# shanjiayao/PTT

Measured on AMD Instinct MI355X. Metric: tracklet frames/sec (hot path: PointNet++ SA stack + Point-Track-Transformer blocks), higher is better.
Workload: dtype f32

## Files before the change

include/ptt_hip.h:

```cpp
#ifndef PTT_HIP_H
#define PTT_HIP_H

#include <stddef.h>
#include <stdint.h>

#ifdef __cplusplus
extern "C" {
#endif

#define PTT_ABI_VERSION 21

enum {
    PTT_OK = 0,
    PTT_EINVAL = -1,
    PTT_EUNSUPPORTED = -2,
    PTT_ELAUNCH = -3,
    PTT_EWORKSPACE = -4
};

typedef void* ptt_stream_t;

int ptt_version(void);
const char* ptt_error_name(int code);
const char* ptt_last_error_string(void);

int ptt_fps_f32(const float* xyz, int B, int N, int npoint, int32_t* idx_out,
                ptt_stream_t stream);
int ptt_fps_ws_f32(const float* xyz, int B, int N, int npoint, int32_t* idx_out, float* workspace,
                   size_t workspace_elems, ptt_stream_t stream);

int ptt_gather_f32(const float* feat, const int32_t* idx, int B, int C, int N, int M,
                   float* out, ptt_stream_t stream);
int ptt_gather_grad_f32(const float* grad_out, const int32_t* idx, int B, int C, int N,
// ... 81 lines not shown
    float radius;
    int32_t ns, M, normalize_xyz, pro_relu;
} ptt_row_job;
int ptt_row_jobs_f32(const ptt_row_job* jobs, int n_jobs, ptt_stream_t stream);

typedef struct ptt_sa_desc {
    const float* xyz;
    const float* new_xyz;
    const int32_t* idx;
    const float* feat;
    int64_t feat_sb, feat_sc, feat_sn;
    float* out;
    int64_t out_sb, out_sc, out_sm;
    int B, N, M, nsample, C;
    float radius;
    int use_xyz;
    int normalize_xyz;
    int n_layers;
    ptt_sa_layer layers[PTT_SA_MAX_LAYERS];
    const float* l0_point_term;
    const float* l0_xyz_weight;
    int l0_channels;
    int l0_relu;
} ptt_sa_desc;

int ptt_sa_fused_fwd_f32(const ptt_sa_desc* d, ptt_stream_t stream);

typedef struct ptt_xcorr_desc {
    const float* cos_t;
    const float* P;
    const float* w_sim;
    const float* scale0;
    const float* shift0;
    float* out;
    int64_t out_sb, out_sc, out_sn;
    float* sim_out;
    int B, Ns, Nt, C0;
    int n_layers;
    ptt_sa_layer layers[PTT_SA_MAX_LAYERS];
    int32_t split; int64_t out_sh;
    const float* search_feat; const float* templ_feat;
    int64_t s_sb, s_sn, t_sb, t_sn;
    int C; float eps;
} ptt_xcorr_desc;

int ptt_xcorr_fused_fwd_f32(const ptt_xcorr_desc* d, ptt_stream_t stream);

int ptt_cosine_map_f32(const float* search_feat, int64_t s_sb, int64_t s_sn, int64_t s_sc, const float* templ_feat,
                       int64_t t_sb, int64_t t_sn, int64_t t_sc, int B, int Ns, int Nt, int C, float eps,
// ... 299 lines not shown
```

ptt_amd/_lib.py:

```python
import ctypes
import os
from ctypes import POINTER, Structure, c_char_p, c_double, c_float, c_int, c_int32, c_int64, c_longlong, c_size_t, c_uint32, c_void_p

_HERE = os.path.dirname(os.path.abspath(__file__))
LIB_PATH = os.path.join(_HERE, "lib", "libptt_hip.so")

PTT_SA_MAX_LAYERS = 4
ABI_VERSION = 21

EXPORTS = [
    "ptt_version", "ptt_error_name", "ptt_last_error_string",
    "ptt_fps_f32", "ptt_fps_ws_f32", "ptt_spatial_order_f32", "ptt_ball_query_grid_workspace", "ptt_ball_query_grid_f32",
    "ptt_centres_ball_query_grid_f32", "ptt_gather_f32", "ptt_gather_grad_f32", "ptt_select_centres_f32", "ptt_ball_query_f32",
    "ptt_group_f32", "ptt_group_grad_f32", "ptt_scatter_add_det_workspace", "ptt_scatter_add_det_f32",
    "ptt_knn_f32", "ptt_knn_rel_f32",
    "ptt_packed_weight_elems", "ptt_pack_weight_f32", "ptt_pack_weight_rot_f32", "ptt_linear_f32",
    "ptt_sa_fused_fwd_f32", "ptt_xcorr_fused_fwd_f32", "ptt_cosine_map_f32", "ptt_pt_attn_pair_f32",
    "ptt_crop_compact_f32", "ptt_regularize_f32", "ptt_mt19937_fill", "ptt_select_box_f32",
    "ptt_track_crop_bounds", "ptt_track_box_by_offset",
    "ptt_bn_stats_workspace", "ptt_bn_stats_f32", "ptt_bn_apply_f32", "ptt_bn_bwd_f32", "ptt_pool_rows_f32",
    "ptt_pool_rows_bwd_f32", "ptt_linear_wgrad_workspace", "ptt_linear_wgrad_f32",
    "ptt_pack_weight_strided_f32", "ptt_linear_batched_f32", "ptt_softmax_rows_f32",
    "ptt_gather_rows_f32", "ptt_scatter_csr_i32", "ptt_scatter_rows_csr_f32",
    "ptt_pt_pair_input_f32", "ptt_pt_attn_train_fwd_f32", "ptt_pt_attn_train_bwd_f32", "ptt_linear_act_in_f32",
    "ptt_centres_ball_query_f32",
    "ptt_bn_sums_f64", "ptt_bn_finish_f64", "ptt_bn_bwd_sums_f64", "ptt_bn_bwd_apply_f32",
    "ptt_rows_mlp_f32",
    "ptt_rows_gemm_supported", "ptt_rows_gemm_stat_chunks", "ptt_rows_gemm_f32", "ptt_rows_gemm_masked_f32", "ptt_bn_finish_partials_f32",
    "ptt_bn_sums_partials_f64", "ptt_linear_wgrad2_workspace", "ptt_linear_wgrad2_f32",
    "ptt_bn_bwd_pooled_f32", "ptt_bn_bwd_pooled_sums_f64", "ptt_bn_bwd_pooled_apply_f32",
    "ptt_pt_pair_input_ld_f32", "ptt_pt_attn_fwd_ld_f32",
    "ptt_rows_gemm_bnbwd_f32", "ptt_bn_bwd_from_partials_f32", "ptt_bn_bwd_sums_partials_f64",
    "ptt_bn_bwd_consts_f32", "ptt_bn_bwd_pooled_consts_f32", "ptt_rows_gemm_bnbwd_fused_supported", "ptt_rows_gemm_bnbwd_fused_f32",
    "ptt_bn_update_running_f32", "ptt_xcorr_z0_f32", "ptt_xcorr_z0_stat_chunks", "ptt_xcorr_z0_stats_f32", "ptt_xcorr_z0_bnbwd_f32", "ptt_xcorr_z0_bwd_workspace", "ptt_xcorr_z0_bwd_f32",
    "ptt_bn_stats_train_f32", "ptt_bn_finish_partials_train_f32", "ptt_pack_weights_f32",
    "ptt_sa_z0_rows_f32",
    "ptt_row_jobs_f32", "ptt_point_jobs_f32", "ptt_fps_ball_knn_f32", "ptt_crop_compact_host_f32", "ptt_crop_regularize_f32", "ptt_colsum_workspace", "ptt_colsum_f32", "ptt_rows_gemm_pool_supported", "ptt_rows_gemm_pool_f32", "ptt_pool_select_f32", "ptt_sa_z0_rows_stat_chunks", "ptt_sa_z0_rows_stats_f32",
    "ptt_track_losses_f32", "ptt_track_losses_bwd_f32", "ptt_adam_chunk_elems", "ptt_adam_clip_step_f32", "ptt_adam_clip_step_dev_f32",
    "ptt_linear_wgrad_partials_f32", "ptt_linear_wgrad2_partials_f32", "ptt_colsum_partials_f32", "ptt_grad_finish_f32",
    "ptt_rows_gemm_rsum16_supported", "ptt_rows_gemm_rsum16_f32", "ptt_scatter_rows_csr_sub_f32",
    "ptt_unit_rows_f32", "ptt_cos_bwd_rows_f32", "ptt_track_select_update", "ptt_sa_z0_bnbwd_workspace", "ptt_sa_z0_bnbwd_f32",
]
PTT_MAX_SEGMENTS = 4


class CropJob(Structure):
    _fields_ = [("points", c_void_p), ("ld", c_int64),
                ("lo1", c_double * 3), ("hi1", c_double * 3), ("trans", c_double * 3), ("rot", c_double * 9),
                ("lo2", c_double * 3), ("hi2", c_double * 3),
                ("out", c_void_p), ("count", c_void_p), ("n_points", c_int32), ("capacity", c_int32),
                ("label_out", c_void_p), ("ltrans", c_double * 3), ("lrot", c_double * 9), ("llo", c_double * 3), ("lhi", c_double * 3)]


class RegularizeJob(Structure):
    _fields_ = [("seg", c_void_p * PTT_MAX_SEGMENTS), ("seg_count", c_void_p * PTT_MAX_SEGMENTS),
                ("seg_capacity", c_int32 * PTT_MAX_SEGMENTS), ("out", c_void_p), ("info", c_void_p),
                ("n_seg", c_int32), ("input_size", c_int32)]



class BnTrainTail(Structure):
    _fields_ = [("gamma", c_void_p), ("beta", c_void_p), ("act_a", c_void_p), ("act_b", c_void_p),
                ("running_mean", c_void_p), ("running_var", c_void_p), ("num_batches_tracked", c_void_p), ("momentum", c_float)]

# ... 45 lines not shown

class GradSegment(Structure):
    _fields_ = [("dst", c_int64), ("n", c_int32), ("cols", c_int32), ("ld", c_int32), ("job0", c_int32), ("njobs", c_int32), ("out", c_int32),
                ("vec", c_int32), ("reserved", c_int32)]


class AdamHyper(Structure):
    _fields_ = [("beta1", c_float), ("beta2", c_float), ("one_minus_beta1", c_float), ("one_minus_beta2", c_float), ("eps", c_float), ("step_size", c_float), ("bias2_sqrt", c_float),
                ("weight_decay", c_float), ("max_norm", c_float), ("write_clipped", c_int32)]


class SaLayer(Structure):
    _fields_ = [("Wpacked", c_void_p), ("scale", c_void_p), ("shift", c_void_p),
                ("Cin", c_int), ("Cout", c_int), ("relu", c_int)]


class SaDesc(Structure):
    _fields_ = [("xyz", c_void_p), ("new_xyz", c_void_p), ("idx", c_void_p), ("feat", c_void_p),
                ("feat_sb", c_int64), ("feat_sc", c_int64), ("feat_sn", c_int64),
                ("out", c_void_p), ("out_sb", c_int64), ("out_sc", c_int64), ("out_sm", c_int64),
                ("B", c_int), ("N", c_int), ("M", c_int), ("nsample", c_int), ("C", c_int),
                ("radius", c_float), ("use_xyz", c_int), ("normalize_xyz", c_int), ("n_layers", c_int),
                ("layers", SaLayer * PTT_SA_MAX_LAYERS),
                ("l0_point_term", c_void_p), ("l0_xyz_weight", c_void_p), ("l0_channels", c_int), ("l0_relu", c_int)]


class XcorrDesc(Structure):
    _fields_ = [("cos_t", c_void_p), ("P", c_void_p), ("w_sim", c_void_p), ("scale0", c_void_p), ("shift0", c_void_p),
                ("out", c_void_p), ("out_sb", c_int64), ("out_sc", c_int64), ("out_sn", c_int64),
                ("sim_out", c_void_p),
                ("B", c_int), ("Ns", c_int), ("Nt", c_int), ("C0", c_int),
                ("n_layers", c_int), ("layers", SaLayer * PTT_SA_MAX_LAYERS),
                ("split", c_int32), ("out_sh", c_int64), ("search_feat", c_void_p), ("templ_feat", c_void_p),
                ("s_sb", c_int64), ("s_sn", c_int64), ("t_sb", c_int64), ("t_sn", c_int64), ("C", c_int), ("eps", c_float)]


class AttnDesc(Structure):
    _fields_ = [("xyz", c_void_p), ("rel", c_void_p), ("knn", c_void_p), ("qkv", c_void_p),
                ("Wd1p", c_void_p), ("Wd2p", c_void_p), ("bd2", c_void_p),
                ("Wg1p", c_void_p), ("bg1", c_void_p), ("Wg2p", c_void_p), ("bg2", c_void_p),
                ("res", c_void_p), ("attn", c_void_p),
                ("B", c_int), ("N", c_int), ("k", c_int), ("D", c_int), ("order", c_void_p)]


_lib = None


# ... 107 lines not shown
        "ptt_bn_bwd_pooled_apply_f32": [vp, i, vp, i, vp, i, vp, vp, vp, vp, vp, vp, i, i, vp, i, vp, vp, vp],
        "ptt_row_jobs_f32": [POINTER(RowJob), i, vp],
        "ptt_point_jobs_f32": [POINTER(PointJob), i, vp],
        "ptt_fps_ball_knn_f32": [vp, i, i, i, f, i, i, vp, vp, vp, vp, vp, vp, vp],
    }
    for name, args in sigs.items():
        fn = getattr(lib, name)
        fn.restype = c_int
        fn.argtypes = args
    lib.ptt_packed_weight_elems.restype = c_size_t
    lib.ptt_packed_weight_elems.argtypes = [i, i]
    lib.ptt_scatter_add_det_workspace.restype = c_size_t
    lib.ptt_scatter_add_det_workspace.argtypes = [i, i, i]
    lib.ptt_ball_query_grid_workspace.restype = c_size_t
    lib.ptt_ball_query_grid_workspace.argtypes = [i, i]
    lib.ptt_bn_stats_workspace.restype = c_size_t
    lib.ptt_bn_stats_workspace.argtypes = [i, i]
    lib.ptt_linear_wgrad_workspace.restype = c_size_t
    lib.ptt_linear_wgrad_workspace.argtypes = [i, i, i]
    lib.ptt_xcorr_z0_bwd_workspace.restype = c_size_t
    lib.ptt_xcorr_z0_bwd_workspace.argtypes = [i, i, i]
    lib.ptt_sa_z0_bnbwd_workspace.restype = c_size_t
    lib.ptt_sa_z0_bnbwd_workspace.argtypes = [c_longlong, i]
    lib.ptt_adam_chunk_elems.restype = c_int
    lib.ptt_adam_chunk_elems.argtypes = []
    lib.ptt_colsum_workspace.restype = c_size_t
    lib.ptt_colsum_workspace.argtypes = [i, i]
    lib.ptt_linear_wgrad2_workspace.restype = c_size_t
    lib.ptt_linear_wgrad2_workspace.argtypes = [i, i, i]


def lib():
    global _lib
    if _lib is None:
        if not os.path.exists(LIB_PATH):
            raise RuntimeError(
                "ptt_amd: %s is missing — build it with `python -m ptt_amd.build` "
                "(hipcc --offload-arch=gfx950); there is no CPU fallback" % LIB_PATH)
        import torch
        try:
            loaded = ctypes.CDLL(LIB_PATH)
        except OSError as e:
            raise RuntimeError("ptt_amd: cannot load %s: %s" % (LIB_PATH, e))
        _declare(loaded)
        if loaded.ptt_version() != ABI_VERSION:
            raise RuntimeError("ptt_amd: %s has ABI version %d, this package expects %d — rebuild it with "
# ... 11 lines not shown
```

ptt_amd/csrc/mfma_ops.hip:

```cpp
#include <math.h>
#include <stdlib.h>
#include <string.h>
#include "common.h"
#include "mfma_common.h"

#ifndef PTT_PAIR_PF
#define PTT_PAIR_PF 1
#endif
#ifndef PTT_GATHER_BATCH
#define PTT_GATHER_BATCH 16
#endif
#ifndef PTT_SA_WAVES
#define PTT_SA_WAVES 2
#endif

namespace ptt {

#ifdef PTT_DEV
#define PTT_STAMP(i) do { if (p.dbg && threadIdx.x == 0 && blockIdx.x < 4096) p.dbg[blockIdx.x * 8 + (i)] = __builtin_readcyclecounter(); } while (0)
#else
#define PTT_STAMP(i) do { } while (0)
#endif

__device__ __forceinline__ void stagger_second_slot(int first_wave_blocks, int quanta) {
// ... 399 lines not shown
    const float sc = p.scale ? p.scale[col] : 1.f;
    const float sh = p.shift ? p.shift[col] : 0.f;
#pragma unroll
    for (int r = 0; r < 16; ++r) {
        const int gr = row0 + tile_row(r, half);
        if (gr >= p.rows) continue;
        float y = (acc[r] + Rs[(cw * 16 + r) * 64 + lane]) * sc + sh;
        if (p.relu) y = fmaxf(y, 0.f);
        if (p.residual) y += p.residual[(size_t)gr * p.ldr + col];
        p.out[(size_t)gr * p.ldo + col] = y;
    }
}

struct SaLayerDev { const float* Wp; const float* scale; const float* shift; int Cin, Cout, relu, nkb, NT; };
struct SaParams {
    const float* xyz; const float* new_xyz; const int32_t* idx; const float* feat; float* out;
    long long fsb, fsc, fsn, osb, osc, osm;
    int B, N, M, C, use_xyz, normalize, n_layers, ldk, K0, first_wave, stagger, vec_gather;
    int tiles, chunk;
    int hoist, l0_relu;
    const float* wx;
    float radius;
    long long* dbg;
    SaLayerDev L[PTT_SA_MAX_LAYERS];
};

struct RowsMlpParams {
    const float* X; const float* residual; float* out;
    int rows, K0, ldx, ldr, ldo, n_layers, ldk, vec_in;
    SaLayerDev L[PTT_SA_MAX_LAYERS];
};

__global__ __launch_bounds__(256, 2) void rows_mlp_kernel(RowsMlpParams p) {
    extern __shared__ __attribute__((aligned(16))) float smem[];
    float* Xs = smem;
    const int t = threadIdx.x, lane = t & 63, w = t >> 6, half = lane >> 5;
    const int row0 = blockIdx.x * 32;
    f32x4 pw[3];
    float psh[3];
    auto prefetch = [&](const SaLayerDev& L) {
        const f32x4* bp = reinterpret_cast<const f32x4*>(L.Wp) + (size_t)w * 64 + lane;
#pragma unroll
        for (int u = 0; u < 3; ++u) {
            psh[u] = 0.f;
            if (w + 4 * u < L.NT) {
                pw[u] = bp[(size_t)u * 4 * 64];
// ... 783 lines not shown
            } else {
                float m0 = y[0], m1 = y[8];
#pragma unroll
                for (int r = 1; r < 8; ++r) { m0 = fmaxf(m0, y[r]); m1 = fmaxf(m1, y[8 + r]); }
                m0 = max_halves(m0);
                m1 = max_halves(m1);
                if (L.relu) { m0 = fmaxf(m0, 0.f); m1 = fmaxf(m1, 0.f); }
                if (half == 0) {
                    if (2 * rt < ncentres) {
                        const int c = centre0 + 2 * rt; const int b = c / p.M, mm = c - b * p.M;
                        p.out[b * p.osb + col * p.osc + mm * p.osm] = m0;
                    }
                    if (2 * rt + 1 < ncentres) {
                        const int c = centre0 + 2 * rt + 1; const int b = c / p.M, mm = c - b * p.M;
                        p.out[b * p.osb + col * p.osc + mm * p.osm] = m1;
                    }
                }
            }
        }
    }
    __builtin_amdgcn_wave_barrier();
}

#ifndef PTT_SAL_WGS
#define PTT_SAL_WGS 1
#endif
#ifndef PTT_SAL_WAVES
#define PTT_SAL_WAVES 12
#endif
__global__ __launch_bounds__(64 * PTT_SAL_WAVES) __attribute__((amdgpu_waves_per_eu(PTT_SAL_WAVES * PTT_SAL_WGS / 4)))
void sa_lds_kernel(SaParams p) {
    extern __shared__ __attribute__((aligned(16))) float smem[];
    float* W1 = smem;
    float* W2 = smem + 4096;
    const int t = threadIdx.x, lane = t & 63, half = lane >> 5, col = lane & 31;
    const int w = __builtin_amdgcn_readfirstlane(t >> 6);
    {
        const f32x4* g1 = reinterpret_cast<const f32x4*>(p.L[1].Wp);
        const f32x4* g2 = reinterpret_cast<const f32x4*>(p.L[2].Wp);
        f32x4* s1 = reinterpret_cast<f32x4*>(W1);
        f32x4* s2 = reinterpret_cast<f32x4*>(W2);
        const int nthr = (int)blockDim.x;
        for (int i = t; i < 1024; i += nthr) s1[i] = g1[i];
        for (int i = t; i < 2048; i += nthr) s2[i] = g2[i];
    }
    float* cst = smem + 4096 + 8192 + w * 640 + lane;
#pragma unroll
    for (int u = 0; u < 2; ++u) {
        const f32x4 f = reinterpret_cast<const f32x4*>(p.L[0].Wp)[u * 64 + col];
        const float s0 = p.L[0].shift ? p.L[0].shift[u * 32 + col] : 0.f;
        cst[(0 + u) * 64] = half ? f[1] : f[0];
        cst[(2 + u) * 64] = half ? s0 : f[2];
        cst[(4 + u) * 64] = p.L[1].shift ? p.L[1].shift[u * 32 + col] : 0.f;
    }
#pragma unroll
    for (int u = 0; u < 4; ++u) cst[(6 + u) * 64] = p.L[2].shift ? p.L[2].shift[u * 32 + col] : 0.f;
    const float one_zero = half ? 0.f : 1.f, one_hi = 1.f;
    __syncthreads();
    const int total = p.B * p.M, M = p.M, N = p.N;
    const int gw = logical_block() * ((int)blockDim.x >> 6) + w;
    const int c0 = gw * p.chunk, c1 = min(total, c0 + p.chunk);
    if (c0 >= c1) return;
    const float rdiv = p.normalize ? p.radius : 1.0f;
    const int osb = (int)p.osb, osm = (int)p.osm, osc = (int)p.osc;
    const f32x16 zero16 = {0.f, 0.f, 0.f, 0.f, 0.f, 0.f, 0.f, 0.f, 0.f, 0.f, 0.f, 0.f, 0.f, 0.f, 0.f, 0.f};
    const float* a1p = W1 + lane * 4;
    const float* b2p = W2 + lane * 4;
    const __amdgpu_buffer_rsrc_t rx = weight_rsrc(p.xyz);

    SasCentre ce;
    ce.c = c0; ce.b = c0 / M; ce.m = c0 - ce.b * M;
    int n_cur = p.idx[(size_t)c0 * 32 + col];
    float px, py, pz, cx, cy, cz;
    {
        const size_t flat = (size_t)ce.b * N + n_cur;
        px = p.xyz[flat * 3]; py = p.xyz[flat * 3 + 1]; pz = p.xyz[flat * 3 + 2];
        cx = p.new_xyz[(size_t)c0 * 3]; cy = p.new_xyz[(size_t)c0 * 3 + 1]; cz = p.new_xyz[(size_t)c0 * 3 + 2];
    }
    for (int c = c0; c < c1; ++c) {
        SasCentre nx = ce;
        if (c + 1 < c1) nx.advance(1, M);
        const int n_next = p.idx[(size_t)nx.c * 32 + col];
        f32x4 wa[2], wn[2];
#pragma unroll
        for (int u = 0; u < 2; ++u) wa[u] = *reinterpret_cast<const f32x4*>(a1p + u * 256);
        const float dx = (px - cx) / rdiv, dy = (py - cy) / rdiv, dz = (pz - cz) / rdiv;
        __builtin_amdgcn_sched_barrier(0);
        f32x16 h0[2];
        {
            const float k0 = half ? dy : dx, k1 = half ? one_hi : dz;
#pragma unroll
            for (int u = 0; u < 2; ++u) h0[u] = __builtin_amdgcn_mfma_f32_32x32x2f32(cst[(0 + u) * 64], k0, zero16, 0, 0, 0);
#pragma unroll
            for (int u = 0; u < 2; ++u) h0[u] = __builtin_amdgcn_mfma_f32_32x32x2f32(cst[(2 + u) * 64], k1, h0[u], 0, 0, 0);
#pragma unroll
            for (int u = 0; u < 2; ++u)
#pragma unroll
                for (int r = 0; r < 16; ++r) h0[u][r] = fmaxf(h0[u][r], 0.f);
        }
        f32x16 h1[2];
        f32x4 wb[4], wm[4];
        {
#pragma unroll
            for (int u = 0; u < 2; ++u) h1[u] = __builtin_amdgcn_mfma_f32_32x32x2f32(cst[(4 + u) * 64], one_zero, zero16, 0, 0, 0);
#pragma unroll
// ... 1 lines not shown
                if (kb < 7) {
#pragma unroll
                    for (int u = 0; u < 2; ++u) wn[u] = *reinterpret_cast<const f32x4*>(a1p + ((kb + 1) * 2 + u) * 256);
                } else {
#pragma unroll
                    for (int u = 0; u < 4; ++u) wb[u] = *reinterpret_cast<const f32x4*>(b2p + u * 256);
                }
                __builtin_amdgcn_sched_barrier(0);
#pragma unroll
                for (int j = 0; j < 4; ++j)
#pragma unroll
                    for (int u = 0; u < 2; ++u)
                        h1[u] = __builtin_amdgcn_mfma_f32_32x32x2f32(wa[u][j], h0[kb >> 2][(kb & 3) * 4 + j], h1[u], 0, 0, 0);
                __builtin_amdgcn_sched_barrier(0);
#pragma unroll
                for (int u = 0; u < 2; ++u) wa[u] = wn[u];
            }
#pragma unroll
            for (int u = 0; u < 2; ++u)
#pragma unroll
                for (int r = 0; r < 16; ++r) h1[u][r] = fmaxf(h1[u][r], 0.f);
        }
        {
            const int off = (nx.b * N + n_next) * 12;
            px = __builtin_bit_cast(float, __builtin_amdgcn_raw_buffer_load_b32(rx, off, 0, 0));
            py = __builtin_bit_cast(float, __builtin_amdgcn_raw_buffer_load_b32(rx, off + 4, 0, 0));
            pz = __builtin_bit_cast(float, __builtin_amdgcn_raw_buffer_load_b32(rx, off + 8, 0, 0));
            cx = p.new_xyz[(size_t)nx.c * 3]; cy = p.new_xyz[(size_t)nx.c * 3 + 1]; cz = p.new_xyz[(size_t)nx.c * 3 + 2];
        }
        __builtin_amdgcn_sched_barrier(0);
        {
            f32x16 acc[4];
#pragma unroll
            for (int kb = 0; kb < 8; ++kb) {
                if (kb < 7) {
#pragma unroll
                    for (int u = 0; u < 4; ++u) wm[u] = *reinterpret_cast<const f32x4*>(b2p + ((kb + 1) * 4 + u) * 256);
                }
                __builtin_amdgcn_sched_barrier(0);
#pragma unroll
                for (int j = 0; j < 4; ++j)
#pragma unroll
                    for (int u = 0; u < 4; ++u)
                        acc[u] = __builtin_amdgcn_mfma_f32_32x32x2f32(h1[kb >> 2][(kb & 3) * 4 + j], wb[u][j],
                                                                       (kb == 0 && j == 0) ? zero16 : acc[u], 0, 0, 0);
                __builtin_amdgcn_sched_barrier(0);
#pragma unroll
                for (int u = 0; u < 4; ++u) wb[u] = wm[u];
            }
            float* o = p.out + (ce.b * osb + ce.m * osm);
#pragma unroll
            for (int u = 0; u < 4; ++u) {
                const float mx = sas_pool(acc[u], cst[(6 + u) * 64], p.L[2].relu);
                if (half == 0) o[(u * 32 + col) * osc] = mx;
            }
        }
        ce = nx;
    }
}

template <int NS, int RT>
__global__ __launch_bounds__(256, 2) void sa_wave_kernel(SaParams p) {
    extern __shared__ __attribute__((aligned(16))) float smem[];
    constexpr int CPW = 32 * RT / NS;
    const int t = threadIdx.x, lane = t & 63, w = t >> 6;
    float* Xw = smem + w * 32 * RT * p.ldk;
    const int total_centres = p.B * p.M;
    const int centre0 = (logical_block() * 4 + w) * CPW;
    if (centre0 >= total_centres) return;
    const int ncentres = min(CPW, total_centres - centre0);

#pragma unroll
    for (int rt = 0; rt < RT; ++rt) sa_gather_rows<NS, 32>(p, Xw, rt * 32, centre0, lane);
    __builtin_amdgcn_wave_barrier();

    for (int l = 0; l < p.n_layers; ++l) {
        const SaLayerDev& L = p.L[l];
        const bool last = (l == p.n_layers - 1);
#define PTT_WAVE_LAYER(CTV)                                                                         \
        { if (L.scale) sa_wave_layer<NS, CTV, true, RT>(p, L, last, Xw, lane, centre0, ncentres);       \
// ... 335 lines not shown
        const ptt_sa_layer& s = layers[l];
        const bool last = l == n_layers - 1;
        if (s.Cin != cin) return fail(PTT_EINVAL, "ptt_rows_mlp_f32: layer %d Cin=%d, expected %d", l, s.Cin, cin);
        if (s.Cout <= 0 || s.Cout > (last ? 384 : 256))
            return fail(PTT_EUNSUPPORTED, "ptt_rows_mlp_f32: layer %d Cout=%d (inner layers <= 256, the last <= 384)", l, s.Cout);
        if (!s.Wpacked) return fail(PTT_EINVAL, "ptt_rows_mlp_f32: layer %d has no weights", l);
        SaLayerDev& L = p.L[l];
        L.Wp = s.Wpacked; L.scale = s.scale; L.shift = s.shift; L.Cin = s.Cin; L.Cout = s.Cout; L.relu = s.relu;
        L.nkb = (s.Cin + 7) / 8; L.NT = (s.Cout + 31) / 32;
        if (L.nkb * 8 > maxk) maxk = L.nkb * 8;
        if (!last && L.NT * 32 > maxk) maxk = L.NT * 32;
        cin = s.Cout;
    }
    if (ldo < cin || (residual && ldr < cin)) return fail(PTT_EINVAL, "ptt_rows_mlp_f32: ldo=%d ldr=%d Cout=%d", ldo, ldr, cin);
    p.ldk = maxk + 4;
    p.vec_in = ((K & 3) == 0 && (ldx & 3) == 0 && (reinterpret_cast<uintptr_t>(X) & 15) == 0) ? 1 : 0;
    const int lds = 32 * p.ldk * (int)sizeof(float);
    int rc = set_lds_limit(reinterpret_cast<const void*>(rows_mlp_kernel), lds);
    if (rc) return rc;
    hipLaunchKernelGGL(rows_mlp_kernel, dim3((rows + 31) / 32), dim3(256), lds, as_stream(stream), p);
    return check_launch("rows_mlp_kernel");
}

extern "C" int ptt_sa_fused_fwd_f32(const ptt_sa_desc* d, ptt_stream_t stream) {
    if (!d) return fail(PTT_EINVAL, "ptt_sa_fused_fwd_f32: null descriptor");
    if (d->B < 0 || d->N <= 0 || d->M < 0 || d->C < 0 || d->n_layers < 1 || d->n_layers > PTT_SA_MAX_LAYERS)
        return fail(PTT_EINVAL, "ptt_sa_fused_fwd_f32: B=%d N=%d M=%d C=%d layers=%d", d->B, d->N, d->M, d->C,
                    d->n_layers);
    if (d->nsample != 16 && d->nsample != 32 && d->nsample != 64)
        return fail(PTT_EUNSUPPORTED, "ptt_sa_fused_fwd_f32: nsample=%d (16, 32 and 64 are instantiated)", d->nsample);
    if (d->B == 0 || d->M == 0) return PTT_OK;
    const bool hoist = d->l0_point_term != nullptr;
    if (!d->xyz || !d->new_xyz || !d->idx || !d->out || (!hoist && d->C > 0 && !d->feat))
        return fail(PTT_EINVAL, "ptt_sa_fused_fwd_f32: null pointer");
    if (!d->use_xyz && d->C == 0) return fail(PTT_EINVAL, "ptt_sa_fused_fwd_f32: no xyz and no features");
    if (hoist) {
        const int c0 = d->l0_channels;
        if (!d->use_xyz || !d->l0_xyz_weight || c0 <= 0 || (c0 % 32) != 0 || c0 > 256 ||
            (reinterpret_cast<uintptr_t>(d->l0_point_term) & 15) != 0 ||
            (reinterpret_cast<uintptr_t>(d->l0_xyz_weight) & 15) != 0)
            return fail(PTT_EINVAL, "ptt_sa_fused_fwd_f32: hoisted layer 0 needs use_xyz, 16-byte aligned (B,N,C0) and "
                        "(3,C0) arrays and C0 a multiple of 32 <= 256 (C0=%d)", c0);
    }

    SaParams p;
    p.xyz = d->xyz; p.new_xyz = d->new_xyz; p.idx = d->idx; p.feat = d->feat; p.out = d->out;
// ... 17 lines not shown
        if (s.Cout <= 0 || (s.Cout % 32) != 0 || s.Cout > 256)
            return fail(PTT_EUNSUPPORTED, "ptt_sa_fused_fwd_f32: layer %d Cout=%d must be a multiple of 32 <= 256", l,
                        s.Cout);
        if (!s.Wpacked) return fail(PTT_EINVAL, "ptt_sa_fused_fwd_f32: layer %d has no weights", l);
        SaLayerDev& L = p.L[l];
        L.Wp = s.Wpacked; L.scale = s.scale; L.shift = s.shift; L.Cin = s.Cin; L.Cout = s.Cout; L.relu = s.relu;
        L.nkb = (s.Cin + 7) / 8; L.NT = s.Cout / 32;
        if (L.nkb * 8 > maxk) maxk = L.nkb * 8;
        if (l + 1 < d->n_layers && s.Cout > maxk) maxk = s.Cout;
        cin = s.Cout;
    }
    {
        const unsigned long long lim = 0x7fffffffull, B = (unsigned long long)d->B;
        if (B * d->N * 12ull >= lim || B * d->M * d->nsample * 4ull >= lim || B * d->M * (unsigned long long)cin * 4ull >= lim ||
            B * d->N * (unsigned long long)(p.C > 0 ? p.C : 1) * 4ull >= lim)
            return fail(PTT_EUNSUPPORTED, "ptt_sa_fused_fwd_f32: B=%d N=%d M=%d: an array of this launch exceeds 2 GiB "
                        "(32-bit offsets) — split the batch", d->B, d->N, d->M);
    }
    p.ldk = maxk + 4;
    p.vec_gather = (p.C > 0 && p.fsc == 1 && (p.C & 3) == 0 && p.C <= 256 && (p.fsn & 3) == 0 &&
                    (p.fsb & 3) == 0 && (reinterpret_cast<uintptr_t>(p.feat) & 15) == 0) ? 1 : 0;
    p.first_wave = 1024; p.stagger = dev_switches().sa_stagger;
    p.dbg = dev_switches().stamps;
    const int total_centres = d->B * d->M;
    hipStream_t s = as_stream(stream);
    int rc;
    if (d->C == 0 && d->use_xyz && !hoist && d->nsample == 32 && d->n_layers == 3 && p.L[0].Cout == 64 && p.L[1].Cout == 64 &&
        p.L[2].Cout == 128 && !p.L[0].scale && !p.L[1].scale && !p.L[2].scale && p.L[0].relu && p.L[1].relu &&
        dev_switches().sa_lds) {
        const int waves = 256 * PTT_SAL_WAVES * PTT_SAL_WGS;
        p.chunk = (total_centres + waves - 1) / waves;
        if (dev_switches().sa_lds_chunk > 0 && p.chunk > dev_switches().sa_lds_chunk) p.chunk = dev_switches().sa_lds_chunk;
        const int nw = total_centres * 3 <= 256 * PTT_SAL_WAVES ? 4 : PTT_SAL_WAVES;
        int wgs = (total_centres + p.chunk * nw - 1) / (p.chunk * nw);
        const int lds = (4096 + 8192 + PTT_SAL_WAVES * 640) * (int)sizeof(float);
        if ((rc = set_lds_limit(reinterpret_cast<const void*>(sa_lds_kernel), lds))) return rc;
        hipLaunchKernelGGL(sa_lds_kernel, dim3(wgs), dim3(64 * nw), lds, s, p);
        return check_launch("sa_lds_kernel");
    }
    size_t wbytes = 0;
    bool wave_ok = true;
    for (int l = 0; l < d->n_layers; ++l) {
        wbytes += (size_t)d->layers[l].Cin * d->layers[l].Cout * sizeof(float);
        const int nt = d->layers[l].Cout / 32;
        if (!(nt == 1 || nt == 2 || nt == 4)) wave_ok = false;
    }
    wave_ok = wave_ok && dev_switches().sa_wave;
    if (wave_ok && wbytes <= 64 * 1024 && d->nsample <= 32) {
        const int lds = 4 * 32 * p.ldk * (int)sizeof(float);
        const int cpw = 32 / d->nsample, per_wg = 4 * cpw;
        const dim3 grid((total_centres + per_wg - 1) / per_wg);
        if (d->nsample == 32) {
            if ((rc = set_lds_limit(reinterpret_cast<const void*>(sa_wave_kernel<32, 1>), lds))) return rc;
            hipLaunchKernelGGL((sa_wave_kernel<32, 1>), grid, dim3(256), lds, s, p);
        } else {
            if ((rc = set_lds_limit(reinterpret_cast<const void*>(sa_wave_kernel<16, 1>), lds))) return rc;
            hipLaunchKernelGGL((sa_wave_kernel<16, 1>), grid, dim3(256), lds, s, p);
        }
        return check_launch("sa_wave_kernel");
    }
// ... 128 lines not shown
```

ptt_amd/models/backbones_3d/pointnet2/pointnet2_modules.py:

```python
import os
from typing import List

import torch
import torch.nn as nn
import torch.nn.functional as F

from .... import ops, train_ops
from . import pointnet2_utils
from . import pytorch_utils as pt_utils


class PointnetSAModuleVotes(nn.Module):
    def __init__(self, *, mlp: List[int], radius: float = None, nsample: int = None, bn: bool = True,
                 use_xyz: bool = True, normalize_xyz: bool = False, sample_uniformly: bool = False,
                 sample_method='fps'):
        super().__init__()
        self.radius = radius
        self.nsample = nsample
        self.mlp_module = None
        self.use_xyz = use_xyz
        self.normalize_xyz = normalize_xyz
        self.sample_uniformly = sample_uniformly
        self.grouper = pointnet2_utils.QueryAndGroup(radius, nsample, use_xyz=use_xyz, ret_grouped_xyz=True,
                                                     normalize_xyz=normalize_xyz, sample_uniformly=sample_uniformly,
# ... 128 lines not shown
            else:
                new_xyz, inds64, idx = ops.centres_ball_query(xyz, inds.contiguous(), npoint, self.radius, self.nsample)
            layers, hoist = self._fused_params(xyz.device)
            if hoist is not None and features is not None:
                wf_packed, wx, c0, relu0 = hoist
                rows = features.transpose(1, 2)
                uniform = rows.stride(2) == 1 and rows.stride(0) == rows.shape[1] * rows.stride(1)
                term = ops.linear(rows if uniform else rows.contiguous(), wf_packed, c0, None, layers[0][2], relu=False)
                B, M, ns = xyz.shape[0], npoint, self.nsample
                if (B * M * ns <= ops.ONE_FRAME_MAX_SA_ROWS and ns in (16, 32) and len(layers) == 3 and c0 % 4 == 0 and c0 >= 192):
                    L1, L2 = layers[1], layers[2]
                    h = torch.empty((B * M * ns, L1[4]), dtype=torch.float32, device=xyz.device)
                    ops.row_jobs([ops.row_job(L1[0], L1[4], prologue=3, x=term, idx=idx, xyz=xyz, centres=new_xyz, wx=wx,
                                              radius=self.radius, ns=ns, M=M, N=xyz.shape[1], normalize_xyz=self.normalize_xyz,
                                              pro_relu=relu0, scale=L1[1], shift=L1[2], act=1 if L1[5] else 0, out=h)])
                    pooled = torch.empty((B, M, L2[4]), dtype=torch.float32, device=xyz.device)
                    ops.row_jobs([ops.row_job(L2[0], L2[4], x=h, epilogue=2, ns=ns, M=M, scale=L2[1], shift=L2[2],
                                              act=1 if L2[5] else 0, out=pooled)])
                    return new_xyz, pooled.transpose(1, 2), inds64
                new_features = ops.sa_fused_forward(xyz, new_xyz, idx, None, [L[:6] for L in layers[1:]], self.radius, True,
                                                    self.normalize_xyz, point_major_out=True, l0=(term, wx, relu0))
            else:
                new_features = ops.sa_fused_forward(xyz, new_xyz, idx, features, [L[:6] for L in layers], self.radius,
                                                    self.use_xyz, self.normalize_xyz, point_major_out=True)
            return new_xyz, new_features, inds64

        hoist = (self.use_xyz and not self.sample_uniformly and self.nsample * npoint <= 16384
                 and train_ops.usable(self.mlp_module, xyz if features is None else features)
                 and self.mlp_module[0].conv.weight.shape[0] % 4 == 0)
        if hoist and not xyz.requires_grad and inds.dtype == torch.int32:
            new_xyz, inds64, idx = ops.centres_ball_query(xyz.contiguous(), inds.contiguous(), npoint, self.radius, self.nsample)
            y = train_ops.sa_level_hoisted(xyz, new_xyz, features, idx, self.mlp_module, self.radius, self.normalize_xyz)
            return new_xyz, y, inds64
        xyz_flipped = xyz.transpose(1, 2).contiguous()
        new_xyz = pointnet2_utils.gather_operation(xyz_flipped, inds).transpose(1, 2).contiguous()
        if hoist and features is not None:
            idx = pointnet2_utils.ball_query(self.radius, self.nsample, xyz, new_xyz)
            y = train_ops.sa_level_hoisted(xyz, new_xyz, features, idx, self.mlp_module, self.radius, self.normalize_xyz)
            return new_xyz, y, inds.to(torch.int64)
        grouped_features, grouped_xyz = self.grouper(xyz, new_xyz, features)
        if train_ops.usable(self.mlp_module, grouped_features):
            return new_xyz, train_ops.shared_mlp_pool(grouped_features, self.mlp_module, pool_dim=3), inds.to(torch.int64)
        y = self.mlp_module(grouped_features)
        y = y.max(dim=3)[0]
        return new_xyz, y, inds.to(torch.int64)
```

ptt_amd/ops.py:

```python
import ctypes
import os

import torch

from . import _lib
from ._lib import AttnDesc, SaDesc, SaLayer, XcorrDesc


def _stream():
    return ctypes.c_void_p(torch.cuda.current_stream().cuda_stream)


_timing = None


def start_kernel_timing(names):
    global _timing
    _timing = {n: [] for n in names}


def stop_kernel_timing():
    global _timing
    t, _timing = _timing, None
    torch.cuda.synchronize()
# ... 272 lines not shown
    if residual is not None:
        r2 = residual.reshape(-1, int(cout))
        if r2.stride(1) != 1:
            r2 = r2.contiguous()
    if (scale is None and (rows > 8192 or (rows >= 6144 and int(cout) == 256)) and x2.data_ptr() % 16 == 0 and o2.is_contiguous()
            and _lib.lib().ptt_rows_gemm_supported(rows, K, int(cout), x2.stride(0), int(cout))):
        with torch.cuda.device(x.device), _timed('ptt_linear_f32'):
            _lib.check(_lib.lib().ptt_rows_gemm_f32(_ptr(x2), rows, K, x2.stride(0), None, None, _ptr(wpacked), int(cout), _ptr(shift),
                                                    1 if relu else 0, _ptr(r2), r2.stride(0) if r2 is not None else int(cout),
                                                    _ptr(o2), int(cout), None, 0, _stream()), "ptt_rows_gemm_f32")
        return out
    if rows <= ROW_JOB_MAX_ROWS and 192 <= K <= 1024 and o2.stride(1) == 1:
        row_jobs([row_job(wpacked, cout, x=x2, scale=scale, shift=shift, act=1 if relu else 0, res=r2, out=o2)])
        return out
    with torch.cuda.device(x.device), _timed('ptt_linear_f32'):
        _lib.check(_lib.lib().ptt_linear_f32(
            _ptr(x2), rows, K, x2.stride(0) if rows > 1 else K, _ptr(wpacked), int(cout), _ptr(scale), _ptr(shift),
            1 if relu else 0, _ptr(r2), (r2.stride(0) if (r2 is not None and rows > 1) else int(cout)),
            _ptr(o2), o2.stride(0) if rows > 1 else int(cout), _stream()), "ptt_linear_f32")
    return out


def sa_fused_forward(xyz, new_xyz, idx, features, layers, radius, use_xyz=True, normalize_xyz=False,
                     point_major_out=True, l0=None):
    _chk(xyz, "xyz", torch.float32, 3)
    _chk(new_xyz, "new_xyz", torch.float32, 3)
    _chk(idx, "idx", torch.int32, 3)
    B, N, _ = xyz.shape
    _, M, ns = idx.shape
    d = SaDesc()
    d.xyz, d.new_xyz, d.idx = xyz.data_ptr(), new_xyz.data_ptr(), idx.data_ptr()
    if features is not None:
        if not features.is_cuda or features.dtype != torch.float32 or features.dim() != 3:
            raise RuntimeError("features must be a (B,C,N) float32 device tensor")
        d.feat = features.data_ptr()
        d.feat_sb, d.feat_sc, d.feat_sn = features.stride()
        d.C = features.shape[1]
    else:
        d.feat, d.C = None, 0
    cout = layers[-1][4]
    if point_major_out:
        store = torch.empty((B, M, cout), dtype=torch.float32, device=xyz.device)
        out = store.transpose(1, 2)
    else:
        out = torch.empty((B, cout, M), dtype=torch.float32, device=xyz.device)
    d.out = out.data_ptr()
    d.out_sb, d.out_sc, d.out_sm = out.stride()
    d.B, d.N, d.M, d.nsample = B, N, M, ns
    d.radius, d.use_xyz, d.normalize_xyz = float(radius), int(bool(use_xyz)), int(bool(normalize_xyz))
    d.n_layers = len(layers)
    for i, (wp, sc, sh, cin, co, relu) in enumerate(layers):
        L = d.layers[i]
        L.Wpacked = wp.data_ptr()
        L.scale = sc.data_ptr() if sc is not None else None
        L.shift = sh.data_ptr() if sh is not None else None
        L.Cin, L.Cout, L.relu = int(cin), int(co), int(bool(relu))
    if l0 is not None:
        term, wx, l0_relu = l0
        if features is not None:
            raise RuntimeError("with a hoisted layer 0 the point features are already inside l0[0]")
        _chk(term, "l0 point term", torch.float32, 3)
        _chk(wx, "l0 xyz weight", torch.float32, 2)
        if term.shape[0] != B or term.shape[1] != N or wx.shape[0] != 3 or wx.shape[1] != term.shape[2]:
            raise RuntimeError("l0 point term must be (B,N,C0) and the xyz weight (3,C0)")
        d.l0_point_term, d.l0_xyz_weight = term.data_ptr(), wx.data_ptr()
        d.l0_channels, d.l0_relu = term.shape[2], int(bool(l0_relu))
    with torch.cuda.device(xyz.device), _timed('ptt_sa_fused_fwd_f32'):
        _lib.check(_lib.lib().ptt_sa_fused_fwd_f32(ctypes.byref(d), _stream()), "ptt_sa_fused_fwd_f32")
    return out


def cosine_map(search_feats, templ_feats, eps=1e-8):
    for t_, n_ in ((search_feats, "search_feats"), (templ_feats, "templ_feats")):
        if not isinstance(t_, torch.Tensor) or not t_.is_cuda or t_.dtype != torch.float32 or t_.dim() != 3:
            raise RuntimeError("%s must be a (B,C,N) float32 device tensor" % n_)
    if search_feats.shape[:2] != templ_feats.shape[:2] or search_feats.device != templ_feats.device:
        raise RuntimeError("search_feats and templ_feats must share batch size, channel count and device")
    B, C, Ns = search_feats.shape
    Nt = templ_feats.shape[2]
    out = torch.empty((B, Ns, Nt), dtype=torch.float32, device=search_feats.device)
    ssb, ssc, ssn = search_feats.stride()
    tsb, tsc, tsn = templ_feats.stride()
    with torch.cuda.device(out.device), _timed('ptt_cosine_map_f32'):
        _lib.check(_lib.lib().ptt_cosine_map_f32(search_feats.data_ptr(), ssb, ssn, ssc, templ_feats.data_ptr(), tsb, tsn,
                                                 tsc, B, Ns, Nt, C, float(eps), out.data_ptr(), _stream()),
                   "ptt_cosine_map_f32")
    return out


# ... 1351 lines not shown
```

Baseline: 16080.

## Compact SA first-layer neighbourhoods by distinct point count before fused MLP

Adds a pre-pass kernel that deduplicates each ball-query neighbourhood (padded duplicate indices and coincident points), counts distinct neighbours, and buckets centres into classes of 4/8/16/32 rows in a workspace table. The fused SA LDS kernel gets a compact variant that walks these buckets, packing several small neighbourhoods into one 32-row MFMA tile and max-pooling per group, so less MLP work is spent on duplicate rows. This costs two extra launches (zero and compact), a workspace allocation per call, and a grid-stride schedule. It is enabled for the first SA layer, where features is None.

```diff
diff --git a/include/ptt_hip.h b/include/ptt_hip.h
--- a/include/ptt_hip.h
+++ b/include/ptt_hip.h
@@ -8,7 +8,7 @@
 extern "C" {
 #endif
 
-#define PTT_ABI_VERSION 21
+#define PTT_ABI_VERSION 22
 
 enum {
     PTT_OK = 0,
@@ -136,9 +136,12 @@
     const float* l0_xyz_weight;
     int l0_channels;
     int l0_relu;
+    void* compact_ws;
+    size_t compact_ws_bytes;
 } ptt_sa_desc;
 
 int ptt_sa_fused_fwd_f32(const ptt_sa_desc* d, ptt_stream_t stream);
+size_t ptt_sa_compact_workspace(int B, int M);
 
 typedef struct ptt_xcorr_desc {
     const float* cos_t;
diff --git a/ptt_amd/_lib.py b/ptt_amd/_lib.py
--- a/ptt_amd/_lib.py
+++ b/ptt_amd/_lib.py
@@ -6,7 +6,7 @@
 LIB_PATH = os.path.join(_HERE, "lib", "libptt_hip.so")
 
 PTT_SA_MAX_LAYERS = 4
-ABI_VERSION = 21
+ABI_VERSION = 22
 
 EXPORTS = [
     "ptt_version", "ptt_error_name", "ptt_last_error_string",
@@ -39,7 +39,7 @@
     "ptt_track_losses_f32", "ptt_track_losses_bwd_f32", "ptt_adam_chunk_elems", "ptt_adam_clip_step_f32", "ptt_adam_clip_step_dev_f32",
     "ptt_linear_wgrad_partials_f32", "ptt_linear_wgrad2_partials_f32", "ptt_colsum_partials_f32", "ptt_grad_finish_f32",
     "ptt_rows_gemm_rsum16_supported", "ptt_rows_gemm_rsum16_f32", "ptt_scatter_rows_csr_sub_f32",
-    "ptt_unit_rows_f32", "ptt_cos_bwd_rows_f32", "ptt_track_select_update", "ptt_sa_z0_bnbwd_workspace", "ptt_sa_z0_bnbwd_f32",
+    "ptt_unit_rows_f32", "ptt_cos_bwd_rows_f32", "ptt_track_select_update", "ptt_sa_z0_bnbwd_workspace", "ptt_sa_compact_workspace", "ptt_sa_z0_bnbwd_f32",
 ]
 PTT_MAX_SEGMENTS = 4
 
@@ -131,7 +131,8 @@
                 ("B", c_int), ("N", c_int), ("M", c_int), ("nsample", c_int), ("C", c_int),
                 ("radius", c_float), ("use_xyz", c_int), ("normalize_xyz", c_int), ("n_layers", c_int),
                 ("layers", SaLayer * PTT_SA_MAX_LAYERS),
-                ("l0_point_term", c_void_p), ("l0_xyz_weight", c_void_p), ("l0_channels", c_int), ("l0_relu", c_int)]
+                ("l0_point_term", c_void_p), ("l0_xyz_weight", c_void_p), ("l0_channels", c_int), ("l0_relu", c_int),
+                ("compact_ws", c_void_p), ("compact_ws_bytes", c_size_t)]
 
 
 class XcorrDesc(Structure):
@@ -285,6 +286,8 @@
     lib.ptt_xcorr_z0_bwd_workspace.argtypes = [i, i, i]
     lib.ptt_sa_z0_bnbwd_workspace.restype = c_size_t
     lib.ptt_sa_z0_bnbwd_workspace.argtypes = [c_longlong, i]
+    lib.ptt_sa_compact_workspace.restype = c_size_t
+    lib.ptt_sa_compact_workspace.argtypes = [i, i]
     lib.ptt_adam_chunk_elems.restype = c_int
     lib.ptt_adam_chunk_elems.argtypes = []
     lib.ptt_colsum_workspace.restype = c_size_t
diff --git a/ptt_amd/csrc/mfma_ops.hip b/ptt_amd/csrc/mfma_ops.hip
--- a/ptt_amd/csrc/mfma_ops.hip
+++ b/ptt_amd/csrc/mfma_ops.hip
@@ -445,6 +445,7 @@
     const float* wx;
     float radius;
     long long* dbg;
+    int32_t* cws;
     SaLayerDev L[PTT_SA_MAX_LAYERS];
 };
 
@@ -1274,12 +1275,155 @@
     __builtin_amdgcn_wave_barrier();
 }
 
+constexpr int SAC_HDR = 16;
+struct SacTable {
+    int32_t* ws; int T;
+    __host__ __device__ int32_t* ndist() const { return ws + SAC_HDR; }
+    __host__ __device__ int32_t* list(int k) const { return ws + SAC_HDR + (size_t)(1 + k) * T; }
+    __host__ __device__ int32_t* rows(int k) const { return ws + SAC_HDR + 5 * (size_t)T + (size_t)((4 << k) - 4) * T; }
+    static size_t words(size_t T) { return SAC_HDR + 65 * T; }
+};
+constexpr int SAC_PASSES = 4;
+
+__global__ __launch_bounds__(64) void sa_compact_zero_kernel(int32_t* ws) {
+    if (threadIdx.x < 4) ws[threadIdx.x] = 0;
+}
+
+__global__ __launch_bounds__(256) void sa_compact_kernel(const float* __restrict__ xyz, const int32_t* __restrict__ idx, int N, int M,
+                                                         SacTable tab) {
+    __shared__ int s_cnt[4], s_base[4], s_cls[32], s_pos[32], s_nd[32];
+    __shared__ int s_row[32][32];
+    const int t = threadIdx.x, lane = t & 63, half = lane >> 5, s = lane & 31, w = t >> 6;
+    const int g0 = blockIdx.x * 32, T = tab.T;
+    if (t < 4) s_cnt[t] = 0;
+    __syncthreads();
+    int iv[SAC_PASSES];
+    uint32_t x[SAC_PASSES], y[SAC_PASSES], z[SAC_PASSES];
+#pragma unroll
+    for (int q = 0; q < SAC_PASSES; ++q) iv[q] = idx[(size_t)min(g0 + q * 8 + w * 2 + half, T - 1) * 32 + s];
+#pragma unroll
+    for (int q = 0; q < SAC_PASSES; ++q) {
+        const int b = min(g0 + q * 8 + w * 2 + half, T - 1) / M;
+        const uint32_t* pt = reinterpret_cast<const uint32_t*>(xyz) + ((size_t)b * N + iv[q]) * 3;
+        x[q] = pt[0]; y[q] = pt[1]; z[q] = pt[2];
+    }
+#pragma unroll
+    for (int q = 0; q < SAC_PASSES; ++q) {
+        const int lc = q * 8 + w * 2 + half;
+        const int i0a = __builtin_amdgcn_readlane(iv[q], 0), i0b = __builtin_amdgcn_readlane(iv[q], 32);
+        const int i0 = half ? i0b : i0a;
+        const bool real = s == 0 || iv[q] != i0;
+        const unsigned long long rm = __ballot(real);
+        const int J = 31 - __builtin_clz((uint32_t)rm | (uint32_t)(rm >> 32));
+        int dup = 0;
+        for (int j = 0; j < J; ++j) {
+            const uint32_t xa = __builtin_amdgcn_readlane(x[q], j), xb = __builtin_amdgcn_readlane(x[q], 32 + j);
+            const uint32_t ya = __builtin_amdgcn_readlane(y[q], j), yb = __builtin_amdgcn_readlane(y[q], 32 + j);
+            const uint32_t za = __builtin_amdgcn_readlane(z[q], j), zb = __builtin_amdgcn_readlane(z[q], 32 + j);
+            dup |= (int)(j < s) & (int)(x[q] == (half ? xb : xa)) & (int)(y[q] == (half ? yb : ya)) & (int)(z[q] == (half ? zb : za));
+        }
+        const bool keep = real && !dup;
+        const unsigned long long km = __ballot(keep);
+        const uint32_t m = half ? (uint32_t)(km >> 32) : (uint32_t)km;
+        const int nd = __popc(m);
+        if (keep) s_row[lc][__popc(m & ((1u << s) - 1u))] = iv[q];
+        if (s == 0) {
+            const int k = nd <= 4 ? 0 : nd <= 8 ? 1 : nd <= 16 ? 2 : 3;
+            const bool valid = g0 + lc < T;
+            s_cls[lc] = valid ? k : -1;
+            s_nd[lc] = nd;
+            s_pos[lc] = valid ? atomicAdd(&s_cnt[k], 1) : 0;
+            if (valid) tab.ndist()[g0 + lc] = nd;
+        }
+    }
+    __syncthreads();
+    if (t < 4) s_base[t] = s_cnt[t] ? atomicAdd(&tab.ws[t], s_cnt[t]) : 0;
+    __syncthreads();
+    for (int e = t; e < 32 * 32; e += 256) {
+        const int lc = e >> 5, j = e & 31, k = s_cls[lc];
+        if (k < 0 || j >= (4 << k)) continue;
+        const int q = s_base[k] + s_pos[lc];
+        tab.rows(k)[(size_t)q * (4 << k) + j] = s_row[lc][j < s_nd[lc] ? j : 0];
+        if (j == 0) tab.list(k)[q] = g0 + lc;
+    }
+}
+
 #ifndef PTT_SAL_WGS
 #define PTT_SAL_WGS 1
 #endif
 #ifndef PTT_SAL_WAVES
 #define PTT_SAL_WAVES 12
 #endif
+
+struct SacTile {
+    int k, first, n;
+    __device__ __forceinline__ void at(int j, const int (&tiles)[4], const int (&cnt)[4]) {
+        k = j < tiles[0] ? 0 : j < tiles[1] ? 1 : j < tiles[2] ? 2 : 3;
+        const int j0 = k == 0 ? 0 : k == 1 ? tiles[0] : k == 2 ? tiles[1] : tiles[2];
+        const int nk = k == 0 ? cnt[0] : k == 1 ? cnt[1] : k == 2 ? cnt[2] : cnt[3];
+        first = (j - j0) << (3 - k);
+        n = min(8 >> k, nk - first);
+    }
+    __device__ __forceinline__ void row(const SacTable& tab, int s, int& n_out, int& ball) const {
+        const int cl = s >> (2 + k), inb = cl < n;
+        n_out = tab.rows(k)[(size_t)first * (4 << k) + (inb ? s : (s & ((4 << k) - 1)))];
+        ball = tab.list(k)[first + (inb ? cl : 0)];
+    }
+};
+
+__device__ __forceinline__ void sac_store(const SaParams& p, const SacTile& tc, int ball, const f32x16 (&acc)[4], const float* cst,
+                                          int half, int col, int osb, int osm, int osc) {
+    const int k = tc.k, relu = p.L[2].relu;
+    int ob[8];
+#pragma unroll
+    for (int g = 0; g < 8; ++g) {
+        if (g >= (8 >> k)) break;
+        const int id = __builtin_amdgcn_readlane(ball, g << (2 + k)), b = id / p.M;
+        ob[g] = b * osb + (id - b * p.M) * osm;
+    }
+#pragma unroll
+    for (int u = 0; u < 4; ++u) {
+        const float sh = cst[(6 + u) * 64];
+        float* o = p.out + (u * 32 + col) * osc;
+        const f32x16& a = acc[u];
+        if (k == 3) {
+            const float mx = sas_pool(a, sh, relu);
+            if (half == 0) o[ob[0]] = mx;
+        } else if (k == 2) {
+            float m0 = a[0], m1 = a[8];
+#pragma unroll
+            for (int r = 1; r < 8; ++r) { m0 = fmaxf(m0, a[r]); m1 = fmaxf(m1, a[8 + r]); }
+            m0 = max_halves(m0) + sh; m1 = max_halves(m1) + sh;
+            if (relu) { m0 = fmaxf(m0, 0.f); m1 = fmaxf(m1, 0.f); }
+            if (half < tc.n) o[half ? ob[1] : ob[0]] = half ? m1 : m0;
+        } else {
+            float m[4];
+#pragma unroll
+            for (int q = 0; q < 4; ++q) m[q] = fmaxf(fmaxf(a[4 * q], a[4 * q + 1]), fmaxf(a[4 * q + 2], a[4 * q + 3]));
+            if (k == 1) {
+#pragma unroll
+                for (int q = 0; q < 4; ++q) m[q] = max_halves(m[q]) + sh;
+#pragma unroll
+                for (int i = 0; i < 2; ++i) {
+                    const int g = 2 * half + i;
+                    float v = half ? m[2 + i] : m[i];
+                    if (relu) v = fmaxf(v, 0.f);
+                    if (g < tc.n) o[half ? ob[2 + i] : ob[i]] = v;
+                }
+            } else {
+#pragma unroll
+                for (int q = 0; q < 4; ++q) {
+                    const int g = 2 * q + half;
+                    float v = m[q] + sh;
+                    if (relu) v = fmaxf(v, 0.f);
+                    if (g < tc.n) o[half ? ob[2 * q + 1] : ob[2 * q]] = v;
+                }
+            }
+        }
+    }
+}
+
+template <bool COMPACT>
 __global__ __launch_bounds__(64 * PTT_SAL_WAVES) __attribute__((amdgpu_waves_per_eu(PTT_SAL_WAVES * PTT_SAL_WGS / 4)))
 void sa_lds_kernel(SaParams p) {
     extern __shared__ __attribute__((aligned(16))) float smem[];
@@ -1287,6 +1431,18 @@
     float* W2 = smem + 4096;
     const int t = threadIdx.x, lane = t & 63, half = lane >> 5, col = lane & 31;
     const int w = __builtin_amdgcn_readfirstlane(t >> 6);
+    const int total = p.B * p.M, M = p.M, N = p.N;
+    const int nw = (int)blockDim.x >> 6;
+    SacTable tab{p.cws, total};
+    int cnt[4], tiles[4];
+    if constexpr (COMPACT) {
+#pragma unroll
+        for (int k = 0; k < 4; ++k) {
+            cnt[k] = min(max(p.cws[k], 0), total);
+            tiles[k] = (k ? tiles[k - 1] : 0) + ((cnt[k] + (8 >> k) - 1) >> (3 - k));
+        }
+        if (logical_block() >= tiles[3]) return;
+    }
     {
         const f32x4* g1 = reinterpret_cast<const f32x4*>(p.L[1].Wp);
         const f32x4* g2 = reinterpret_cast<const f32x4*>(p.L[2].Wp);
@@ -1309,9 +1465,13 @@
     for (int u = 0; u < 4; ++u) cst[(6 + u) * 64] = p.L[2].shift ? p.L[2].shift[u * 32 + col] : 0.f;
     const float one_zero = half ? 0.f : 1.f, one_hi = 1.f;
     __syncthreads();
-    const int total = p.B * p.M, M = p.M, N = p.N;
-    const int gw = logical_block() * ((int)blockDim.x >> 6) + w;
-    const int c0 = gw * p.chunk, c1 = min(total, c0 + p.chunk);
+    int c0, c1, cstep;
+    if constexpr (COMPACT) {
+        c0 = logical_block() + (int)gridDim.x * w; c1 = tiles[3]; cstep = (int)gridDim.x * nw;
+    } else {
+        const int gw = logical_block() * nw + w;
+        c0 = gw * p.chunk; c1 = min(total, c0 + p.chunk); cstep = 1;
+    }
     if (c0 >= c1) return;
     const float rdiv = p.normalize ? p.radius : 1.0f;
     const int osb = (int)p.osb, osm = (int)p.osm, osc = (int)p.osc;
@@ -1320,19 +1480,35 @@
     const float* b2p = W2 + lane * 4;
     const __amdgpu_buffer_rsrc_t rx = weight_rsrc(p.xyz);
 
-    SasCentre ce;
-    ce.c = c0; ce.b = c0 / M; ce.m = c0 - ce.b * M;
-    int n_cur = p.idx[(size_t)c0 * 32 + col];
+    SasCentre ce{0, 0, 0};
+    SacTile tc{0, 0, 0};
     float px, py, pz, cx, cy, cz;
-    {
+    int g_cur = 0;
+    if constexpr (COMPACT) {
+        tc.at(c0, tiles, cnt);
+        int n_cur;
+        tc.row(tab, col, n_cur, g_cur);
+        const size_t flat = (size_t)(g_cur / M) * N + n_cur;
+        px = p.xyz[flat * 3]; py = p.xyz[flat * 3 + 1]; pz = p.xyz[flat * 3 + 2];
+        cx = p.new_xyz[(size_t)g_cur * 3]; cy = p.new_xyz[(size_t)g_cur * 3 + 1]; cz = p.new_xyz[(size_t)g_cur * 3 + 2];
+    } else {
+        ce.c = c0; ce.b = c0 / M; ce.m = c0 - ce.b * M;
+        const int n_cur = p.idx[(size_t)c0 * 32 + col];
         const size_t flat = (size_t)ce.b * N + n_cur;
         px = p.xyz[flat * 3]; py = p.xyz[flat * 3 + 1]; pz = p.xyz[flat * 3 + 2];
         cx = p.new_xyz[(size_t)c0 * 3]; cy = p.new_xyz[(size_t)c0 * 3 + 1]; cz = p.new_xyz[(size_t)c0 * 3 + 2];
     }
-    for (int c = c0; c < c1; ++c) {
+    for (int c = c0; c < c1; c += cstep) {
         SasCentre nx = ce;
-        if (c + 1 < c1) nx.advance(1, M);
-        const int n_next = p.idx[(size_t)nx.c * 32 + col];
+        SacTile tx = tc;
+        int n_next, g_next;
+        if constexpr (COMPACT) {
+            if (c + cstep < c1) tx.at(c + cstep, tiles, cnt);
+            tx.row(tab, col, n_next, g_next);
+        } else {
+            if (c + 1 < c1) nx.advance(1, M);
+            n_next = p.idx[(size_t)nx.c * 32 + col];
+        }
         f32x4 wa[2], wn[2];
 #pragma unroll
         for (int u = 0; u < 2; ++u) wa[u] = *reinterpret_cast<const f32x4*>(a1p + u * 256);
@@ -1380,11 +1556,12 @@
                 for (int r = 0; r < 16; ++r) h1[u][r] = fmaxf(h1[u][r], 0.f);
         }
         {
-            const int off = (nx.b * N + n_next) * 12;
+            const int g = COMPACT ? g_next : nx.c;
+            const int off = ((COMPACT ? g_next / M : nx.b) * N + n_next) * 12;
             px = __builtin_bit_cast(float, __builtin_amdgcn_raw_buffer_load_b32(rx, off, 0, 0));
             py = __builtin_bit_cast(float, __builtin_amdgcn_raw_buffer_load_b32(rx, off + 4, 0, 0));
             pz = __builtin_bit_cast(float, __builtin_amdgcn_raw_buffer_load_b32(rx, off + 8, 0, 0));
-            cx = p.new_xyz[(size_t)nx.c * 3]; cy = p.new_xyz[(size_t)nx.c * 3 + 1]; cz = p.new_xyz[(size_t)nx.c * 3 + 2];
+            cx = p.new_xyz[(size_t)g * 3]; cy = p.new_xyz[(size_t)g * 3 + 1]; cz = p.new_xyz[(size_t)g * 3 + 2];
         }
         __builtin_amdgcn_sched_barrier(0);
         {
@@ -1406,14 +1583,18 @@
 #pragma unroll
                 for (int u = 0; u < 4; ++u) wb[u] = wm[u];
             }
-            float* o = p.out + (ce.b * osb + ce.m * osm);
-#pragma unroll
-            for (int u = 0; u < 4; ++u) {
-                const float mx = sas_pool(acc[u], cst[(6 + u) * 64], p.L[2].relu);
-                if (half == 0) o[(u * 32 + col) * osc] = mx;
-            }
-        }
-        ce = nx;
+            if constexpr (COMPACT) {
+                sac_store(p, tc, g_cur, acc, cst, half, col, osb, osm, osc);
+            } else {
+                float* o = p.out + (ce.b * osb + ce.m * osm);
+#pragma unroll
+                for (int u = 0; u < 4; ++u) {
+                    const float mx = sas_pool(acc[u], cst[(6 + u) * 64], p.L[2].relu);
+                    if (half == 0) o[(u * 32 + col) * osc] = mx;
+                }
+            }
+        }
+        if constexpr (COMPACT) { tc = tx; g_cur = g_next; } else ce = nx;
     }
 }
 
@@ -1795,6 +1976,11 @@
     return check_launch("rows_mlp_kernel");
 }
 
+extern "C" size_t ptt_sa_compact_workspace(int B, int M) {
+    const long long T = (long long)(B > 0 ? B : 0) * (M > 0 ? M : 0);
+    return SacTable::words((size_t)T) * sizeof(int32_t);
+}
+
 extern "C" int ptt_sa_fused_fwd_f32(const ptt_sa_desc* d, ptt_stream_t stream) {
     if (!d) return fail(PTT_EINVAL, "ptt_sa_fused_fwd_f32: null descriptor");
     if (d->B < 0 || d->N <= 0 || d->M < 0 || d->C < 0 || d->n_layers < 1 || d->n_layers > PTT_SA_MAX_LAYERS)
@@ -1858,6 +2044,7 @@
                     (p.fsb & 3) == 0 && (reinterpret_cast<uintptr_t>(p.feat) & 15) == 0) ? 1 : 0;
     p.first_wave = 1024; p.stagger = dev_switches().sa_stagger;
     p.dbg = dev_switches().stamps;
+    p.cws = nullptr;
     const int total_centres = d->B * d->M;
     hipStream_t s = as_stream(stream);
     int rc;
@@ -1870,8 +2057,23 @@
         const int nw = total_centres * 3 <= 256 * PTT_SAL_WAVES ? 4 : PTT_SAL_WAVES;
         int wgs = (total_centres + p.chunk * nw - 1) / (p.chunk * nw);
         const int lds = (4096 + 8192 + PTT_SAL_WAVES * 640) * (int)sizeof(float);
-        if ((rc = set_lds_limit(reinterpret_cast<const void*>(sa_lds_kernel), lds))) return rc;
-        hipLaunchKernelGGL(sa_lds_kernel, dim3(wgs), dim3(64 * nw), lds, s, p);
+        if (d->compact_ws) {
+            if (d->compact_ws_bytes < ptt_sa_compact_workspace(d->B, d->M) || (reinterpret_cast<uintptr_t>(d->compact_ws) & 15))
+                return fail(PTT_EWORKSPACE, "ptt_sa_fused_fwd_f32: compact_ws needs %zu bytes, 16-byte aligned (got %zu)",
+                            ptt_sa_compact_workspace(d->B, d->M), d->compact_ws_bytes);
+            p.cws = static_cast<int32_t*>(d->compact_ws);
+            hipLaunchKernelGGL(sa_compact_zero_kernel, dim3(1), dim3(64), 0, s, p.cws);
+            if ((rc = check_launch("sa_compact_zero_kernel"))) return rc;
+            hipLaunchKernelGGL(sa_compact_kernel, dim3((total_centres + 31) / 32), dim3(256), 0, s, d->xyz, d->idx, d->N, d->M,
+                               SacTable{p.cws, total_centres});
+            if ((rc = check_launch("sa_compact_kernel"))) return rc;
+            if (wgs > 256 * PTT_SAL_WGS) wgs = 256 * PTT_SAL_WGS;
+            if ((rc = set_lds_limit(reinterpret_cast<const void*>(sa_lds_kernel<true>), lds))) return rc;
+            hipLaunchKernelGGL(sa_lds_kernel<true>, dim3(wgs), dim3(64 * nw), lds, s, p);
+            return check_launch("sa_lds_kernel");
+        }
+        if ((rc = set_lds_limit(reinterpret_cast<const void*>(sa_lds_kernel<false>), lds))) return rc;
+        hipLaunchKernelGGL(sa_lds_kernel<false>, dim3(wgs), dim3(64 * nw), lds, s, p);
         return check_launch("sa_lds_kernel");
     }
     size_t wbytes = 0;
diff --git a/ptt_amd/models/backbones_3d/pointnet2/pointnet2_modules.py b/ptt_amd/models/backbones_3d/pointnet2/pointnet2_modules.py
--- a/ptt_amd/models/backbones_3d/pointnet2/pointnet2_modules.py
+++ b/ptt_amd/models/backbones_3d/pointnet2/pointnet2_modules.py
@@ -174,7 +174,8 @@
                                                     self.normalize_xyz, point_major_out=True, l0=(term, wx, relu0))
             else:
                 new_features = ops.sa_fused_forward(xyz, new_xyz, idx, features, [L[:6] for L in layers], self.radius,
-                                                    self.use_xyz, self.normalize_xyz, point_major_out=True)
+                                                    self.use_xyz, self.normalize_xyz, point_major_out=True,
+                                                    compact=features is None)
             return new_xyz, new_features, inds64
 
         hoist = (self.use_xyz and not self.sample_uniformly and self.nsample * npoint <= 16384
diff --git a/ptt_amd/ops.py b/ptt_amd/ops.py
--- a/ptt_amd/ops.py
+++ b/ptt_amd/ops.py
@@ -318,7 +318,7 @@
 
 
 def sa_fused_forward(xyz, new_xyz, idx, features, layers, radius, use_xyz=True, normalize_xyz=False,
-                     point_major_out=True, l0=None):
+                     point_major_out=True, l0=None, compact=False):
     _chk(xyz, "xyz", torch.float32, 3)
     _chk(new_xyz, "new_xyz", torch.float32, 3)
     _chk(idx, "idx", torch.int32, 3)
@@ -361,6 +361,13 @@
             raise RuntimeError("l0 point term must be (B,N,C0) and the xyz weight (3,C0)")
         d.l0_point_term, d.l0_xyz_weight = term.data_ptr(), wx.data_ptr()
         d.l0_channels, d.l0_relu = term.shape[2], int(bool(l0_relu))
+    if isinstance(compact, torch.Tensor):
+        if not compact.is_cuda or compact.device != xyz.device or not compact.is_contiguous():
+            raise RuntimeError("compact workspace must be a contiguous tensor on %s" % xyz.device)
+        d.compact_ws, d.compact_ws_bytes = compact.data_ptr(), compact.numel() * compact.element_size()
+    elif compact:
+        ws = _ws(_lib.lib().ptt_sa_compact_workspace(B, M), xyz.device)
+        d.compact_ws, d.compact_ws_bytes = ws.data_ptr(), ws.numel() * 8
     with torch.cuda.device(xyz.device), _timed('ptt_sa_fused_fwd_f32'):
         _lib.check(_lib.lib().ptt_sa_fused_fwd_f32(ctypes.byref(d), _stream()), "ptt_sa_fused_fwd_f32")
     return out
```

Measured after the change: 16830, median of 6. +4.6%, better.
